# GoatWu/AdaLog

Hardware: AMD Instinct MI355X
Metric: calib_images_per_sec (higher is better)
Workload: dtype bf16

## Files before the change

adalog_amd/csrc/gram.hip:

```cpp
#include "common.h"
#include "fpcs_tail.h"
#include <stdlib.h>
#include <type_traits>
#include <utility>

namespace {

typedef int v4i __attribute__((ext_vector_type(4)));
typedef int v16i __attribute__((ext_vector_type(16)));

template <typename F, int... I> __device__ __forceinline__ void static_for_impl(F&& f, std::integer_sequence<int, I...>) {
    (f(std::integral_constant<int, I>{}), ...);
}
template <int N, typename F> __device__ __forceinline__ void static_for(F&& f) { static_for_impl(f, std::make_integer_sequence<int, N>{}); }

constexpr int RLIMBS = 4;
constexpr int CLIMBS = 8;
constexpr int RFIX_BITS = 29;

__global__ __launch_bounds__(256) void k_gram_pack_xt(const float* __restrict__ x, int T, int K, int64_t ldx, const float* __restrict__ sa,
                                                      const float* __restrict__ za, float qmax, int8_t* __restrict__ xt, int64_t Tp) {
#pragma clang fp contract(off)
    __shared__ uint32_t tile[64][17];
    const int tid = threadIdx.x, tx = tid & 15, ty = tid >> 4;
    const int m0 = blockIdx.x * 64, k0 = blockIdx.y * 64;
    const float s = sa[0], z = rintf(za[0]), inv = 1.0f / s;
#pragma unroll
    for (int i = 0; i < 4; ++i) {
        const int m = m0 + ty + 16 * i, k = k0 + 4 * tx;
        uint32_t pk = 0;
        if (m < T && k < K) {
            const float4 v = *reinterpret_cast<const float4*>(x + (int64_t)m * ldx + k);
            const float e[4] = {v.x, v.y, v.z, v.w};
#pragma unroll
            for (int j = 0; j < 4; ++j) {
                const int q = (int)(uni_bin_fast(e[j], s, inv, z, qmax) - z);
                pk |= ((uint32_t)(q & 0xff)) << (8 * j);
            }
        }
        tile[ty + 16 * i][tx] = pk;
    }
    __syncthreads();
    const int c = tid >> 2, part = tid & 3;
    if (k0 + c < K) {
        uint32_t o[4];
#pragma unroll
        for (int w = 0; w < 4; ++w) {
            uint32_t u = 0;
#pragma unroll
            for (int j = 0; j < 4; ++j) {
                const uint32_t d = tile[part * 16 + w * 4 + j][c >> 2];
                u |= ((d >> (8 * (c & 3))) & 0xffu) << (8 * j);
            }
            o[w] = u;
        }
        *reinterpret_cast<uint4*>(xt + (int64_t)(k0 + c) * Tp + m0 + part * 16) = make_uint4(o[0], o[1], o[2], o[3]);
    }
}

__device__ __forceinline__ double block_sum_d(double v, double* sm) {
#pragma unroll
    for (int o = 32; o > 0; o >>= 1) v += __shfl_xor(v, o);
    const int w = threadIdx.x >> 6;
    __syncthreads();
    if ((threadIdx.x & 63) == 0) sm[w] = v;
    __syncthreads();
    return (sm[0] + sm[1]) + (sm[2] + sm[3]);
}

__global__ __launch_bounds__(256) void k_gram_rmax(const float* __restrict__ ref_t, int T, int chunk, const float* __restrict__ bias,
                                                   unsigned int* __restrict__ amax) {
#pragma clang fp contract(off)
    __shared__ float smf[4];
    const int o = blockIdx.x, tid = threadIdx.x;
    const int m0 = blockIdx.y * chunk, m1 = min(T, m0 + chunk);
    const float* r = ref_t + (int64_t)o * T;
    const float b = bias ? bias[o] : 0.0f;
    float am = 0.0f;
    for (int m = m0 + tid; m < m1; m += 256) am = fmaxf(am, fabsf(r[m] - b));
#pragma unroll
    for (int d = 32; d > 0; d >>= 1) am = fmaxf(am, __shfl_xor(am, d));
    if ((tid & 63) == 0) smf[tid >> 6] = am;
    __syncthreads();
    if (tid == 0) {
        am = fmaxf(fmaxf(smf[0], smf[1]), fmaxf(smf[2], smf[3]));
        if (am == am) atomicMax(amax + o, __float_as_uint(am));
    }
}

__global__ __launch_bounds__(256) void k_gram_rfix(const float* __restrict__ ref_t, int T, int64_t Tp, int O, int chunk, int nchunk,
                                                   const float* __restrict__ bias, const unsigned int* __restrict__ amax,
                                                   int8_t* __restrict__ rl, double* __restrict__ s0p, double* __restrict__ cscl) {
#pragma clang fp contract(off)
    __shared__ double smd[4];
    const int o = blockIdx.x, tid = threadIdx.x;
    const int m0 = blockIdx.y * chunk, m1 = (int)min((int64_t)Tp, (int64_t)m0 + chunk);
    const float* r = ref_t + (int64_t)o * T;
    const float b = bias ? bias[o] : 0.0f;
    const float am = __uint_as_float(amax[o]);
    int e = 0;
    if (am > 0.0f && am < 3.0e38f) e = RFIX_BITS - ilogbf(am);
    const double sc = ldexp(1.0, e);
    double acc = 0.0;
    int8_t* l0 = rl + (int64_t)o * Tp;
    const int64_t plane = (int64_t)O * Tp;
    for (int m = m0 + tid; m < m1; m += 256) {
        int v = 0;
        if (m < T) v = (int)rint((double)(r[m] - b) * sc);
        acc += (double)v * (double)v;
        int rest = v;
#pragma unroll
        for (int l = 0; l < RLIMBS; ++l) {
            const int d = (int)(int8_t)(rest & 0xff);
            l0[l * plane + m] = (int8_t)d;
            rest = (rest - d) >> 8;
        }
    }
    const double tot = block_sum_d(acc, smd);
    if (tid == 0) {
        s0p[(int64_t)o * nchunk + blockIdx.y] = ldexp(tot, -2 * e);
        if (blockIdx.y == 0) cscl[o] = ldexp(1.0, -e);
    }
}

#include "gram_mm.inc"

__global__ __launch_bounds__(256) void k_gram_fin_g(const int* __restrict__ part, int splits, int K, int NL, int8_t* __restrict__ gfrag) {
    const int64_t idx = (int64_t)blockIdx.x * 256 + threadIdx.x;
    if (idx >= (int64_t)K * K) return;
    const int col = (int)(idx % K), slot = (int)(idx / K);
    const int kt = slot >> 5, rp = slot & 31;
    const int row = 32 * kt + 16 * ((rp >> 2) & 1) + 4 * (rp >> 3) + (rp & 3);
    long long g = 0;
    for (int z = 0; z < splits; ++z) g += (long long)part[((int64_t)z * K + row) * K + col];
    const int nj = K >> 5, jt = col >> 5, h = (col >> 4) & 1, e = col & 15;
    long long rest = g;
    for (int l = 0; l < NL; ++l) {
        const int d = (int)(int8_t)(rest & 0xff);
        gfrag[((((int64_t)l * nj + kt) * nj + jt) * 64 + (rp + 32 * h)) * 16 + e] = (int8_t)d;
        rest = (rest - d) >> 8;
    }
}

__global__ __launch_bounds__(256) void k_gram_fin_c(const int* __restrict__ part, int splits, int O, int K, int8_t* __restrict__ clim,
                                                    const double* __restrict__ s0p, int nchunk, double* __restrict__ s0) {
    const int64_t idx = (int64_t)blockIdx.x * 256 + threadIdx.x;
    if (idx < O) {
        double t = 0.0;
        for (int ch = 0; ch < nchunk; ++ch) t += s0p[idx * nchunk + ch];
        s0[idx] = t;
    }
    if (idx >= (int64_t)O * K) return;
    const int o = (int)(idx / K), k = (int)(idx % K);
    long long c = 0;
    for (int z = 0; z < splits; ++z)
#pragma unroll
        for (int l = 0; l < RLIMBS; ++l) c += ((long long)part[((int64_t)z * RLIMBS * O + (int64_t)l * O + o) * K + k]) << (8 * l);
    long long rest = c;
#pragma unroll
    for (int l = 0; l < CLIMBS; ++l) {
        const int d = (int)(int8_t)(rest & 0xff);
        clim[((int64_t)o * CLIMBS + l) * K + k] = (int8_t)d;
        rest = (rest - d) >> 8;
    }
}

template <int OFF> __device__ __forceinline__ v4i gram_rd(uint32_t addr) {
    v4i r;
    asm volatile("ds_read_b128 %0, %1 offset:%2" : "=v"(r) : "v"(addr), "n"(OFF));
    return r;
}
template <int OFF> __device__ __forceinline__ v4i gram_rd_after(uint32_t addr, v16i& tie) {
    v4i r;
    asm volatile("ds_read_b128 %0, %2 offset:%3" : "=v"(r), "+v"(tie) : "v"(addr), "n"(OFF));
    return r;
}
template <int N> __device__ __forceinline__ void gram_wait(v4i& f) {
    if constexpr (N >= 2) asm volatile("s_waitcnt lgkmcnt(2)" : "+v"(f));
    else if constexpr (N == 1) asm volatile("s_waitcnt lgkmcnt(1)" : "+v"(f));
    else asm volatile("s_waitcnt lgkmcnt(0)" : "+v"(f));
}

struct GramScoreArgs {
    const float* W; int64_t ldw; int O, K, P;
    const float* scale; const float* zp;
    const int8_t* gfrag; int NL;
    const int8_t* clim;
    const double* s0; const double* cscl;
    const float* sa;
    double norm;
    float qmax, tie;
    float* scores;
    int nblk;
    long long* timeline;
};

template <int NJ, int NB, bool BIG, bool TIE, int COOP = -1>
__device__ __forceinline__ void gram_pass(const GramScoreArgs& p, uint8_t* lds, int blk0, int w, int lane, float sa, int stamp_slot) {
    constexpr bool CO = COOP >= 0;
    constexpr int QN = CO ? NJ / 4 : NJ;
    constexpr int J0 = CO ? COOP * (NJ / 4) : 0;
    static_assert(!CO || (NJ % 4 == 0 && NB >= 1), "the cooperative pass splits NJ four ways");
    constexpr int NPW = (NJ + 3) / 4;
    constexpr int NRING = 4;
    constexpr int NBA = NB > 0 ? NB : 1;
    const int c = lane & 31, h = lane >> 5;
    const int PB = p.P >> 5;
    const int npanel = NJ * p.NL;
#define GRAM_STAMP(i_) do { if (p.timeline && stamp_slot >= 0 && w == 0 && lane == 0) p.timeline[stamp_slot * 8 + (i_)] = (long long)__builtin_readcyclecounter(); } while (0)
    GRAM_STAMP(0);

    v4i bf[NBA][NJ];
    int orow[NBA];
    float sig[NBA];
    uint8_t* stage = lds + (CO ? 0 : w * (NJ * 1024)) + lane * 16;
    __syncthreads();
    {
#pragma clang fp contract(off)
        static_for<NB>([&](auto bc) {
            constexpr int b = decltype(bc)::value;
            const int blk = blk0 + b;
            const int o = blk / PB, cand = (blk - o * PB) * 32 + c;
            orow[b] = o;
            const int64_t gpi = (int64_t)cand * p.O + o;
            const float gs = p.scale[gpi], gz = rintf(p.zp[gpi]);
            sig[b] = sa * gs;
            const float ginv = __builtin_amdgcn_rcpf(gs);
            const float glo = 128.0f - gz, ghi = 128.0f + (p.qmax - gz);
            const float* __restrict__ wr = p.W + (int64_t)o * p.ldw + 16 * h;
            uint8_t* stb = stage + (CO ? b * (NJ * 1024) : 0);
            float4 nx[4];
#pragma unroll
            for (int j = 0; j < 4; ++j) nx[j] = *reinterpret_cast<const float4*>(wr + 32 * J0 + 4 * j);
#pragma unroll 1
            for (int jt = J0; jt < J0 + QN; ++jt) {
                float xv[16];
#pragma unroll
                for (int j = 0; j < 4; ++j) { xv[4 * j] = nx[j].x; xv[4 * j + 1] = nx[j].y; xv[4 * j + 2] = nx[j].z; xv[4 * j + 3] = nx[j].w; }
                {
                    const int jn = min(jt + 1, NJ - 1);
#pragma unroll
                    for (int j = 0; j < 4; ++j) nx[j] = *reinterpret_cast<const float4*>(wr + 32 * jn + 4 * j);
                }
                float kq[16], dm = 0.0f;
#pragma unroll
                for (int e = 0; e < 16; ++e) {
                    const float t = xv[e] * ginv;
                    kq[e] = rintf(t);
                    dm = fmaxf(dm, fabsf(t - kq[e]));
                }
                if (__builtin_expect(dm > p.tie, 0)) {
#pragma unroll
                    for (int e = 0; e < 16; ++e) kq[e] = rintf(xv[e] / gs);
                }
                v4i pk;
#pragma unroll
                for (int j = 0; j < 4; ++j) {
                    int u = 0;
#pragma unroll
                    for (int e = 0; e < 4; ++e)
                        u = sdwa_rne_byte(u, __builtin_amdgcn_fmed3f(kq[4 * j + e], glo - 128.0f, ghi - 128.0f), 12582912.0f, e);
                    pk[j] = u;
                }
                *reinterpret_cast<v4i*>(stb + jt * 1024) = pk;
            }
            if constexpr (!CO)
                static_for<NJ>([&](auto jtc) { bf[b][decltype(jtc)::value] = *reinterpret_cast<const v4i*>(stb + decltype(jtc)::value * 1024); });
        });
        if constexpr (CO) {
            __syncthreads();
            static_for<NB>([&](auto bc) {
                constexpr int b = decltype(bc)::value;
                static_for<NJ>([&](auto jtc) {
                    bf[b][decltype(jtc)::value] = *reinterpret_cast<const v4i*>(stage + (b * NJ + decltype(jtc)::value) * 1024);
                });
            });
        }
    }
    GRAM_STAMP(1);

    double lin[NBA];
    static_for<NB>([&](auto bc) {
        constexpr int b = decltype(bc)::value;
        v16i acc;
#pragma unroll
        for (int e = 0; e < 16; ++e) acc[e] = 0;
        const int8_t* cr = p.clim + ((int64_t)orow[b] * CLIMBS + (c & 7)) * p.K + 16 * h;
        static_for<QN>([&](auto jtc) {
            constexpr int jt = J0 + decltype(jtc)::value;
            v4i a = *reinterpret_cast<const v4i*>(cr + 32 * jt);
            if (c >= CLIMBS) a = v4i{0, 0, 0, 0};
            acc = __builtin_amdgcn_mfma_i32_32x32x32_i8(a, bf[b][jt], acc, 0, 0, 0);
        });
        double v = 0.0;
#pragma unroll
        for (int j = 0; j < 4; ++j) v += (double)acc[j] * (h ? 4294967296.0 : 1.0) * (double)(1 << (8 * j));
        v += __shfl_xor(v, 32);
        lin[b] = v;
    });
    GRAM_STAMP(2);

    double quad[NBA];
#pragma unroll
    for (int b = 0; b < NBA; ++b) quad[b] = 0.0;
    v4i stg[NPW];
    auto fetch = [&](int pn) {
        const int pc = min(pn, npanel - 1);
        const int8_t* src = p.gfrag + (int64_t)pc * NJ * 1024;
#pragma unroll
        for (int i = 0; i < NPW; ++i) {
            const int piece = min(w + 4 * i, NJ - 1);
            stg[i] = *reinterpret_cast<const v4i*>(src + (int64_t)piece * 1024 + lane * 16);
        }
    };
    auto stash = [&](int pn) {
        uint8_t* dst = lds + (pn % NRING) * (NJ * 1024);
#pragma unroll
        for (int i = 0; i < NPW; ++i) {
            const int piece = min(w + 4 * i, NJ - 1);
            *reinterpret_cast<v4i*>(dst + piece * 1024 + lane * 16) = stg[i];
        }
    };
    __syncthreads();
    fetch(0); stash(0);
    fetch(1); stash(1);
    fetch(2);
    int kt = 0;
    double sh = 1.0;
#pragma unroll 1
    for (int pn = 0; pn < npanel; ++pn) {
        __syncthreads();
        if (pn + 2 < npanel) stash(pn + 2);
        fetch(pn + 3);
        if constexpr (NB > 0) {
            const uint8_t* pan = lds + (pn % NRING) * (NJ * 1024) + lane * 16;
            v16i acc[NB];
#pragma unroll
            for (int b = 0; b < NB; ++b)
#pragma unroll
                for (int e = 0; e < 16; ++e) acc[b][e] = 0;
            constexpr int AD = QN < 3 ? QN : 3;
            v4i af[AD];
            const uint32_t pa = (uint32_t)(uintptr_t)pan;
            static_for<AD>([&](auto ic) { af[decltype(ic)::value] = gram_rd<(J0 + decltype(ic)::value) * 1024>(pa); });
            static_for<QN>([&](auto jtc) {
                constexpr int ji = decltype(jtc)::value, jt = J0 + ji;
                constexpr int left = (QN - 1 - ji) < (AD - 1) ? (QN - 1 - ji) : (AD - 1);
                gram_wait<left>(af[ji % AD]);
                static_for<NB>([&](auto bc) {
                    constexpr int b = decltype(bc)::value;
                    acc[b] = __builtin_amdgcn_mfma_i32_32x32x32_i8(af[ji % AD], bf[b][jt], acc[b], 0, 0, 0);
                });
                if constexpr (ji + AD < QN) {
                    if constexpr (TIE) af[ji % AD] = gram_rd_after<(jt + AD) * 1024>(pa, acc[NB - 1]);
                    else af[ji % AD] = gram_rd<(jt + AD) * 1024>(pa);
                }
            });
            static_for<NB>([&](auto bc) {
                constexpr int b = decltype(bc)::value;
                v4i wv = bf[b][0];
                switch (kt) {
#define GRAM_CASE(i_) case i_: if constexpr ((i_) < NJ) wv = bf[b][(i_) < NJ ? (i_) : 0]; break;
                    GRAM_CASE(1) GRAM_CASE(2) GRAM_CASE(3) GRAM_CASE(4) GRAM_CASE(5) GRAM_CASE(6) GRAM_CASE(7) GRAM_CASE(8)
                    GRAM_CASE(9) GRAM_CASE(10) GRAM_CASE(11) GRAM_CASE(12) GRAM_CASE(13) GRAM_CASE(14) GRAM_CASE(15) GRAM_CASE(16)
                    GRAM_CASE(17) GRAM_CASE(18) GRAM_CASE(19) GRAM_CASE(20) GRAM_CASE(21) GRAM_CASE(22) GRAM_CASE(23)
#undef GRAM_CASE
                    default: break;
                }
                constexpr int GRP = BIG ? 4 : 16;
#pragma unroll
                for (int g0 = 0; g0 < 16; g0 += GRP) {
                    int ts = 0;
#pragma unroll
                    for (int e = g0; e < g0 + GRP; ++e) {
                        const int we = __builtin_amdgcn_sbfe(wv[e >> 2], 8 * (e & 3), 8);
                        ts += __mul24(acc[b][e], we);
                    }
                    quad[b] += (double)ts * sh;
                }
            });
        }
        if (++kt == NJ) { kt = 0; sh *= 256.0; }
    }
    GRAM_STAMP(3);

    if constexpr (CO) {
        double* red = reinterpret_cast<double*>(lds);
        __syncthreads();
        static_for<NB>([&](auto bc) {
            constexpr int b = decltype(bc)::value;
            red[((w * NB + b) * 2 + 0) * 64 + lane] = quad[b];
            red[((w * NB + b) * 2 + 1) * 64 + lane] = lin[b];
        });
        __syncthreads();
        if (w == 0) {
            static_for<NB>([&](auto bc) {
                constexpr int b = decltype(bc)::value;
                double q = 0.0, l = 0.0;
#pragma unroll
                for (int ww = 0; ww < 4; ++ww) { q += red[((ww * NB + b) * 2 + 0) * 64 + lane]; l += red[((ww * NB + b) * 2 + 1) * 64 + lane]; }
                quad[b] = q; lin[b] = l;
            });
        }
    }
    if (!CO || w == 0) {
        static_for<NB>([&](auto bc) {
            constexpr int b = decltype(bc)::value;
            const double q = quad[b] + __shfl_xor(quad[b], 32);
            const int o = orow[b];
            const double s = (double)sig[b];
            const double tot = p.s0[o] - 2.0 * s * (lin[b] * p.cscl[o]) + s * s * q;
            const int blk = blk0 + b;
            const int cand = (blk - o * PB) * 32 + c;
            if (h == 0) p.scores[(int64_t)cand * p.O + o] = (float)(-p.norm * tot);
        });
    }
    GRAM_STAMP(4);
#undef GRAM_STAMP
}

template <int NJ, int CB, bool BIG, int WGS_PER_CU>
__global__ __launch_bounds__(256, WGS_PER_CU) void k_gram_score(GramScoreArgs p) {
#if defined(__HIP_DEVICE_COMPILE__)
    extern __shared__ __attribute__((aligned(16))) uint8_t lds[];
    const int tid = threadIdx.x, lane = tid & 63;
    const int w = __builtin_amdgcn_readfirstlane(tid >> 6);
    const int nwg = gridDim.x;
    const int b_begin = (int)(((int64_t)p.nblk * blockIdx.x) / nwg), b_end = (int)(((int64_t)p.nblk * (blockIdx.x + 1)) / nwg);
    const float sa = p.sa[0];
    int pass_no = 0;
    for (int pass0 = b_begin; pass0 < b_end; pass0 += 4 * CB, ++pass_no) {
        const int n = min(4 * CB, b_end - pass0);
        const int slot = pass_no < 2 ? (int)blockIdx.x * 2 + pass_no : -1;
        if constexpr (NJ % 4 == 0 && NJ >= 8 && NJ != 16) {
            if (n <= CB) {
#define GRAM_COOP(NBV)                                                                                            \
                do {                                                                                              \
                    if (w == 0) gram_pass<NJ, NBV, BIG, WGS_PER_CU == 2, 0>(p, lds, pass0, w, lane, sa, slot);     \
                    else if (w == 1) gram_pass<NJ, NBV, BIG, WGS_PER_CU == 2, 1>(p, lds, pass0, w, lane, sa, slot); \
                    else if (w == 2) gram_pass<NJ, NBV, BIG, WGS_PER_CU == 2, 2>(p, lds, pass0, w, lane, sa, slot); \
                    else gram_pass<NJ, NBV, BIG, WGS_PER_CU == 2, 3>(p, lds, pass0, w, lane, sa, slot);            \
                } while (0)
                if (n == 1) GRAM_COOP(1);
                else if (CB >= 2 && n == 2) GRAM_COOP((CB >= 2 ? 2 : 1));
                else if (CB >= 3 && n == 3) GRAM_COOP((CB >= 3 ? 3 : 1));
                else if (CB >= 4 && n == 4) GRAM_COOP((CB >= 4 ? 4 : 1));
#undef GRAM_COOP
                continue;
            }
        }
        const int nbw = n / 4 + (w < (n & 3) ? 1 : 0);
        const int blk0 = pass0 + w * (n / 4) + min(w, n & 3);
        if (nbw == CB) gram_pass<NJ, CB, BIG, WGS_PER_CU == 2>(p, lds, blk0, w, lane, sa, slot);
        else if (nbw == 0) gram_pass<NJ, 0, BIG, WGS_PER_CU == 2>(p, lds, blk0, w, lane, sa, slot);
        else if (nbw == 1) gram_pass<NJ, 1, BIG, WGS_PER_CU == 2>(p, lds, blk0, w, lane, sa, slot);
        else if (CB > 2 && nbw == 2) gram_pass<NJ, (CB > 2 ? 2 : 1), BIG, WGS_PER_CU == 2>(p, lds, blk0, w, lane, sa, slot);
        else if (CB > 3 && nbw == 3) gram_pass<NJ, (CB > 3 ? 3 : 1), BIG, WGS_PER_CU == 2>(p, lds, blk0, w, lane, sa, slot);
    }
#endif
}

struct GramPlan {
    int T, O, K, NJ, NL;
    int64_t Tp;
    int steps_total, sg_steps, sg_splits, sc_steps, sc_splits, r_chunk, r_nchunk;
    int64_t off_gfrag, off_clim, off_s0, off_cscl, off_xt, off_rl, off_gpart, off_cpart, off_amax, off_s0p, total;
    bool ok;
};

static int g_limbs(int64_t T, int a_bits) {
    const double gmax = (double)T * (double)((1 << a_bits) - 1) * (double)((1 << a_bits) - 1);
    double cover = 127.0;
    for (int L = 1; L <= 7; ++L) {
        if (gmax <= cover) return L;
        cover = cover * 256.0 + 127.0;
    }
    return 8;
}

__global__ __launch_bounds__(256) void k_gram_sum_g(const int* __restrict__ part, int splits, int K, long long* __restrict__ gsum) {
    const int64_t idx = (int64_t)blockIdx.x * 256 + threadIdx.x;
    if (idx >= (int64_t)K * K) return;
    long long g = 0;
    for (int z = 0; z < splits; ++z) g += (long long)part[(int64_t)z * K * K + idx];
    gsum[idx] = g;
}

__global__ __launch_bounds__(256) void k_gram_sum_c(const int* __restrict__ part, int splits, int O, int K, long long* __restrict__ csum,
                                                    const double* __restrict__ s0p, int nchunk, double* __restrict__ s0) {
    const int64_t idx = (int64_t)blockIdx.x * 256 + threadIdx.x;
    if (idx < O) {
        double t = 0.0;
        for (int ch = 0; ch < nchunk; ++ch) t += s0p[idx * nchunk + ch];
        s0[idx] = t;
    }
    if (idx >= (int64_t)O * K) return;
    const int o = (int)(idx / K), k = (int)(idx % K);
    long long c = 0;
    for (int z = 0; z < splits; ++z)
#pragma unroll
        for (int l = 0; l < RLIMBS; ++l) c += ((long long)part[((int64_t)z * RLIMBS * O + (int64_t)l * O + o) * K + k]) << (8 * l);
    csum[idx] = c;
}

__global__ __launch_bounds__(256) void k_gram_limbs_g(const long long* __restrict__ gsum, int K, int NL, int8_t* __restrict__ gfrag) {
    const int64_t idx = (int64_t)blockIdx.x * 256 + threadIdx.x;
    if (idx >= (int64_t)K * K) return;
    const int col = (int)(idx % K), slot = (int)(idx / K);
    const int kt = slot >> 5, rp = slot & 31;
    const int row = 32 * kt + 16 * ((rp >> 2) & 1) + 4 * (rp >> 3) + (rp & 3);
    const int nj = K >> 5, jt = col >> 5, h = (col >> 4) & 1, e = col & 15;
    long long rest = gsum[(int64_t)row * K + col];
    for (int l = 0; l < NL; ++l) {
        const int d = (int)(int8_t)(rest & 0xff);
        gfrag[((((int64_t)l * nj + kt) * nj + jt) * 64 + (rp + 32 * h)) * 16 + e] = (int8_t)d;
        rest = (rest - d) >> 8;
    }
}

__global__ __launch_bounds__(256) void k_gram_limbs_c(const long long* __restrict__ csum, int O, int K, int8_t* __restrict__ clim,
                                                      const double* __restrict__ s0_in, const unsigned int* __restrict__ amax,
                                                      double* __restrict__ s0, double* __restrict__ cscl) {
    const int64_t idx = (int64_t)blockIdx.x * 256 + threadIdx.x;
    if (idx < O) {
        s0[idx] = s0_in[idx];
        const float am = __uint_as_float(amax[idx]);
        int e = 0;
        if (am > 0.0f && am < 3.0e38f) e = RFIX_BITS - ilogbf(am);
        cscl[idx] = ldexp(1.0, -e);
    }
    if (idx >= (int64_t)O * K) return;
    const int o = (int)(idx / K), k = (int)(idx % K);
    long long rest = csum[idx];
#pragma unroll
    for (int l = 0; l < CLIMBS; ++l) {
        const int d = (int)(int8_t)(rest & 0xff);
        clim[((int64_t)o * CLIMBS + l) * K + k] = (int8_t)d;
        rest = (rest - d) >> 8;
    }
}

static int64_t al256(int64_t v) { return (v + 255) / 256 * 256; }

static int pick_steps(int steps_total, int tiles, int target_waves) {
    int splits = (target_waves + tiles - 1) / tiles;
    if (splits < 1) splits = 1;
    int per = (steps_total + splits - 1) / splits;
    if (per < 4) per = 4;
    if (per > 512) per = 512;
    if (per > steps_total) per = steps_total;
    return per;
}

constexpr int MM_BI = 4, MM_BJ = 4;

static GramPlan gram_plan(int T, int O, int K, int a_bits) {
    GramPlan g{};
    g.T = T; g.O = O; g.K = K;
    g.ok = T >= 1 && O >= 1 && K >= 32 && K % 32 == 0 && a_bits >= 2 && a_bits <= 7 && (int64_t)RLIMBS * O < ((int64_t)1 << 30);
    if (!g.ok) return g;
    g.NJ = K / 32;
    g.NL = g_limbs(T, a_bits);
    g.Tp = ((int64_t)T + 127) / 128 * 128;
    g.steps_total = (int)(g.Tp / 128);
    const int tk = (K + 32 * MM_BJ - 1) / (32 * MM_BJ);
    const int tg = ((K + 32 * MM_BI - 1) / (32 * MM_BI)) * tk, tc = ((RLIMBS * O + 32 * MM_BI - 1) / (32 * MM_BI)) * tk;
    g.sg_steps = pick_steps(g.steps_total, tg, 512);
    g.sg_splits = (g.steps_total + g.sg_steps - 1) / g.sg_steps;
    g.sc_steps = pick_steps(g.steps_total, tc, 512);
    g.sc_splits = (g.steps_total + g.sc_steps - 1) / g.sc_steps;
    g.r_chunk = 8192;
    g.r_nchunk = (int)((g.Tp + g.r_chunk - 1) / g.r_chunk);
    int64_t off = 0;
    g.off_gfrag = off; off += al256((int64_t)g.NL * K * K);
    g.off_clim = off; off += al256((int64_t)O * CLIMBS * K);
    g.off_s0 = off; off += al256((int64_t)O * 8);
    g.off_cscl = off; off += al256((int64_t)O * 8);
    g.off_amax = off; off += al256((int64_t)O * 4);
    g.off_s0p = off; off += al256((int64_t)O * g.r_nchunk * 8);
    g.off_xt = off; off += al256((int64_t)K * g.Tp);
    g.off_rl = off; off += al256((int64_t)RLIMBS * O * g.Tp);
    g.off_gpart = off; off += al256((int64_t)g.sg_splits * K * K * 4);
    g.off_cpart = off; off += al256((int64_t)g.sc_splits * RLIMBS * O * K * 4);
    g.total = off;
    return g;
}

static bool nj_supported(int nj) { return nj == 1 || nj == 2 || nj == 3 || nj == 4 || nj == 6 || nj == 8 || nj == 12 || nj == 16 || nj == 24; }

}

extern "C" int adalog_gram_supported(int T, int O, int K, int a_bits, int w_bits, int P) {
    const GramPlan g = gram_plan(T, O, K, a_bits);
    if (!g.ok || !nj_supported(g.NJ) || w_bits < 2 || w_bits > 7 || P < 32 || P % 32 != 0) return 0;
    const int64_t wq = (1 << w_bits) - 1;
    if ((int64_t)128 * wq * K >= (1 << 23)) return 0;
    if ((w_bits > 4 ? 4 : 16) * 128 * wq * wq * K >= ((int64_t)1 << 31)) return 0;
    if ((int64_t)O * P / 32 >= ((int64_t)1 << 30)) return 0;
    return 1;
}

extern "C" int adalog_gram_ok(int T, int O, int K, int a_bits, int w_bits, int P) {
    if (!adalog_gram_supported(T, O, K, a_bits, w_bits, P)) return 0;
    return (int64_t)g_limbs(T, a_bits) * K * 2 <= T ? 1 : 0;
}

extern "C" int adalog_gram_limbs(int T, int a_bits) { return (T >= 1 && a_bits >= 2 && a_bits <= 7) ? g_limbs(T, a_bits) : -1; }

extern "C" int64_t adalog_gram_workspace_bytes(int T, int O, int K, int a_bits) {
    const GramPlan g = gram_plan(T, O, K, a_bits);
    return g.ok ? g.total : -1;
}

extern "C" int adalog_gram_build(const float* x, int T, int K, int64_t ldx, const float* sa, const float* za, int a_bits,
                                 const float* ref_t, int O, const float* bias, void* ws, int64_t ws_bytes, void* stream) {
    ADALOG_ARG_CHECK(x && sa && za && ref_t && ws, "gram_build: null pointer");
    const GramPlan g = gram_plan(T, O, K, a_bits);
    ADALOG_ARG_CHECK(g.ok && nj_supported(g.NJ), "gram_build: shape not supported (adalog_gram_supported)");
    ADALOG_ARG_CHECK(ws_bytes >= g.total, "gram_build: workspace too small");
    ADALOG_ARG_CHECK(ldx >= K && ldx % 4 == 0 && ((uintptr_t)x & 15) == 0 && ((uintptr_t)ws & 255) == 0, "gram_build: x rows / workspace must be aligned");
    hipStream_t st = (hipStream_t)stream;
    uint8_t* base = (uint8_t*)ws;
    int8_t* xt = (int8_t*)(base + g.off_xt);
    int8_t* rl = (int8_t*)(base + g.off_rl);
    int* gpart = (int*)(base + g.off_gpart);
    int* cpart = (int*)(base + g.off_cpart);
    unsigned int* amax = (unsigned int*)(base + g.off_amax);
    double* s0p = (double*)(base + g.off_s0p);
    {
        const hipError_t me = hipMemsetAsync(amax, 0, (size_t)O * 4, st);
        if (me != hipSuccess) { adalog_set_error("adalog_gram_build (clear)", me); return (int)me; }
    }
    hipLaunchKernelGGL(k_gram_pack_xt, dim3((unsigned)(g.Tp / 64), (unsigned)((K + 63) / 64)), dim3(256), 0, st, x, T, K, ldx, sa, za,
                       (float)((1 << a_bits) - 1), xt, g.Tp);
    hipLaunchKernelGGL(k_gram_rmax, dim3((unsigned)O, (unsigned)g.r_nchunk), dim3(256), 0, st, ref_t, T, g.r_chunk, bias, amax);
    hipLaunchKernelGGL(k_gram_rfix, dim3((unsigned)O, (unsigned)g.r_nchunk), dim3(256), 0, st, ref_t, T, g.Tp, O, g.r_chunk, g.r_nchunk, bias,
                       amax, rl, s0p, (double*)(base + g.off_cscl));
    const unsigned tk = (unsigned)((K + 32 * MM_BJ - 1) / (32 * MM_BJ));
    hipLaunchKernelGGL(k_i8mm, dim3((unsigned)((K + 32 * MM_BI - 1) / (32 * MM_BI)), tk, (unsigned)g.sg_splits), dim3(256), 0, st,
                       xt, xt, K, K, g.Tp, g.sg_steps, g.steps_total, gpart);
    hipLaunchKernelGGL(k_i8mm, dim3((unsigned)((RLIMBS * O + 32 * MM_BI - 1) / (32 * MM_BI)), tk, (unsigned)g.sc_splits), dim3(256), 0,
                       st, rl, xt, RLIMBS * O, K, g.Tp, g.sc_steps, g.steps_total, cpart);
    hipLaunchKernelGGL(k_gram_fin_g, dim3((unsigned)(((int64_t)K * K + 255) / 256)), dim3(256), 0, st, gpart, g.sg_splits, K, g.NL,
                       (int8_t*)(base + g.off_gfrag));
    hipLaunchKernelGGL(k_gram_fin_c, dim3((unsigned)(((int64_t)O * K + 255) / 256)), dim3(256), 0, st, cpart, g.sc_splits, O, K,
                       (int8_t*)(base + g.off_clim), s0p, g.r_nchunk, (double*)(base + g.off_s0));
    ADALOG_LAUNCH_CHECK("adalog_gram_build");
    return 0;
}

extern "C" int adalog_gram_amax(const float* ref_t, int T, int O, const float* bias, unsigned int* amax, void* stream) {
    ADALOG_ARG_CHECK(ref_t && amax && T >= 1 && O >= 1, "gram_amax: bad arguments");
    hipStream_t st = (hipStream_t)stream;
    const hipError_t me = hipMemsetAsync(amax, 0, (size_t)O * 4, st);
    if (me != hipSuccess) { adalog_set_error("adalog_gram_amax (clear)", me); return (int)me; }
    const int chunk = 8192, nchunk = (T + chunk - 1) / chunk;
    hipLaunchKernelGGL(k_gram_rmax, dim3((unsigned)O, (unsigned)nchunk), dim3(256), 0, st, ref_t, T, chunk, bias, amax);
    ADALOG_LAUNCH_CHECK("adalog_gram_amax");
    return 0;
}

extern "C" int adalog_gram_build_sums(const float* x, int T, int K, int64_t ldx, const float* sa, const float* za, int a_bits,
                                      const float* ref_t, int O, const float* bias, const unsigned int* amax, long long* gsum,
                                      long long* csum, double* s0, void* ws, int64_t ws_bytes, void* stream) {
    ADALOG_ARG_CHECK(x && sa && za && ref_t && amax && gsum && csum && s0 && ws, "gram_build_sums: null pointer");
    const GramPlan g = gram_plan(T, O, K, a_bits);
    ADALOG_ARG_CHECK(g.ok, "gram_build_sums: shape not supported");
    ADALOG_ARG_CHECK(ws_bytes >= g.total, "gram_build_sums: workspace too small (adalog_gram_workspace_bytes of the LOCAL shape)");
    ADALOG_ARG_CHECK(ldx >= K && ldx % 4 == 0 && ((uintptr_t)x & 15) == 0 && ((uintptr_t)ws & 255) == 0, "gram_build_sums: x rows / workspace must be aligned");
    hipStream_t st = (hipStream_t)stream;
    uint8_t* base = (uint8_t*)ws;
    int8_t* xt = (int8_t*)(base + g.off_xt);
    int8_t* rl = (int8_t*)(base + g.off_rl);
    int* gpart = (int*)(base + g.off_gpart);
    int* cpart = (int*)(base + g.off_cpart);
    double* s0p = (double*)(base + g.off_s0p);
    hipLaunchKernelGGL(k_gram_pack_xt, dim3((unsigned)(g.Tp / 64), (unsigned)((K + 63) / 64)), dim3(256), 0, st, x, T, K, ldx, sa, za,
                       (float)((1 << a_bits) - 1), xt, g.Tp);
    hipLaunchKernelGGL(k_gram_rfix, dim3((unsigned)O, (unsigned)g.r_nchunk), dim3(256), 0, st, ref_t, T, g.Tp, O, g.r_chunk, g.r_nchunk, bias,
                       amax, rl, s0p, (double*)(base + g.off_cscl));
    const unsigned tk = (unsigned)((K + 32 * MM_BJ - 1) / (32 * MM_BJ));
    hipLaunchKernelGGL(k_i8mm, dim3((unsigned)((K + 32 * MM_BI - 1) / (32 * MM_BI)), tk, (unsigned)g.sg_splits), dim3(256), 0, st,
                       xt, xt, K, K, g.Tp, g.sg_steps, g.steps_total, gpart);
    hipLaunchKernelGGL(k_i8mm, dim3((unsigned)((RLIMBS * O + 32 * MM_BI - 1) / (32 * MM_BI)), tk, (unsigned)g.sc_splits), dim3(256), 0,
                       st, rl, xt, RLIMBS * O, K, g.Tp, g.sc_steps, g.steps_total, cpart);
    hipLaunchKernelGGL(k_gram_sum_g, dim3((unsigned)(((int64_t)K * K + 255) / 256)), dim3(256), 0, st, gpart, g.sg_splits, K, gsum);
    hipLaunchKernelGGL(k_gram_sum_c, dim3((unsigned)(((int64_t)O * K + 255) / 256)), dim3(256), 0, st, cpart, g.sc_splits, O, K, csum,
                       s0p, g.r_nchunk, s0);
    ADALOG_LAUNCH_CHECK("adalog_gram_build_sums");
    return 0;
}

extern "C" int adalog_gram_build_from_sums(const long long* gsum, const long long* csum, const double* s0, const unsigned int* amax,
                                           int T_total, int O, int K, int a_bits, void* ws, int64_t ws_bytes, void* stream) {
    ADALOG_ARG_CHECK(gsum && csum && s0 && amax && ws, "gram_build_from_sums: null pointer");
    const GramPlan g = gram_plan(T_total, O, K, a_bits);
    ADALOG_ARG_CHECK(g.ok && nj_supported(g.NJ), "gram_build_from_sums: shape not supported (adalog_gram_supported)");
    ADALOG_ARG_CHECK(ws_bytes >= g.total && ((uintptr_t)ws & 255) == 0, "gram_build_from_sums: workspace too small / misaligned");
    hipStream_t st = (hipStream_t)stream;
    uint8_t* base = (uint8_t*)ws;
    hipLaunchKernelGGL(k_gram_limbs_g, dim3((unsigned)(((int64_t)K * K + 255) / 256)), dim3(256), 0, st, gsum, K, g.NL,
                       (int8_t*)(base + g.off_gfrag));
    hipLaunchKernelGGL(k_gram_limbs_c, dim3((unsigned)(((int64_t)O * K + 255) / 256)), dim3(256), 0, st, csum, O, K,
                       (int8_t*)(base + g.off_clim), s0, amax, (double*)(base + g.off_s0), (double*)(base + g.off_cscl));
    ADALOG_LAUNCH_CHECK("adalog_gram_build_from_sums");
    return 0;
}

static long long* g_gram_timeline = nullptr;
extern "C" void adalog_gram_set_timeline(long long* buf) { g_gram_timeline = buf; }

static int device_cus_gram() { return adalog_device_cus(); }

extern "C" int adalog_gram_score_w(const float* W, int O, int K, int64_t ldw, const float* scale, const float* zp, int P, int w_bits,
                                   const void* ws, int T, int a_bits, const float* sa, double norm, float* scores, void* stream) {
    ADALOG_ARG_CHECK(W && scale && zp && ws && sa && scores, "gram_score_w: null pointer");
    ADALOG_ARG_CHECK(adalog_gram_supported(T, O, K, a_bits, w_bits, P), "gram_score_w: shape not supported (adalog_gram_supported)");
    ADALOG_ARG_CHECK(ldw >= K && ldw % 4 == 0 && ((uintptr_t)W & 15) == 0, "gram_score_w: weight rows must be 16-byte aligned");
    const GramPlan g = gram_plan(T, O, K, a_bits);
    ADALOG_ARG_CHECK(g.ok && nj_supported(g.NJ) && P % 32 == 0, "gram_score_w: shape not supported");
    const uint8_t* base = (const uint8_t*)ws;
    GramScoreArgs a{};
    a.W = W; a.ldw = ldw; a.O = O; a.K = K; a.P = P; a.scale = scale; a.zp = zp;
    a.gfrag = (const int8_t*)(base + g.off_gfrag); a.NL = g.NL; a.clim = (const int8_t*)(base + g.off_clim);
    a.s0 = (const double*)(base + g.off_s0); a.cscl = (const double*)(base + g.off_cscl);
    a.sa = sa; a.norm = norm; a.scores = scores;
    a.qmax = (float)((1 << w_bits) - 1);
    const float zone = 6e-7f * (float)(1 << w_bits);
    a.tie = 0.5f - (zone > 1e-5f ? zone : 1e-5f);
    a.nblk = (int)((int64_t)O * P / 32);
    a.timeline = g_gram_timeline;
    const bool big = w_bits > 4;
    hipStream_t st = (hipStream_t)stream;
    const int ncu = device_cus_gram();
    const int rc = adalog_dispatch<1, 2, 3, 4, 6, 8, 12, 16, 24>(g.NJ, [&](auto nj) {
        return adalog_dispatch<true, false>(big, [&](auto bg) {
            constexpr int NJ = decltype(nj)::value, CB = NJ >= 8 ? 2 : 4, WPC = NJ == 24 ? 1 : 2;
            const int wgs = a.nblk < WPC * ncu ? a.nblk : WPC * ncu;
            return adalog_launch<k_gram_score<NJ, CB, decltype(bg)::value, WPC>>("k_gram_score<i8>", 160 * 1024, (unsigned)wgs, 256,
                                                                                 (size_t)4 * NJ * 1024, st, a);
        });
    });
    if (rc) return rc;
    ADALOG_LAUNCH_CHECK("adalog_gram_score_w");
    return 0;
}

extern "C" int adalog_gram_score_w_tail(const float* W, int O, int K, int64_t ldw, const float* scale, const float* zp, int P, int w_bits,
                                        const void* ws, int T, int a_bits, const float* sa, double norm, float* scores,
                                        const adalog_fpcs_tail* tail, void* stream) {
    const char* why = fpcs::tail_problem(tail, P);
    ADALOG_ARG_CHECK(why == nullptr, why);
    const int rc = adalog_gram_score_w(W, O, K, ldw, scale, zp, P, w_bits, ws, T, a_bits, sa, norm, scores, stream);
    if (rc || !tail) return rc;
    return adalog_topk_next_tail(scores, P, O, tail, nullptr, stream);
}
```

Measured before the change: 38.11.

## Stream Gram panels via buffer-to-LDS DMA in grouped double buffers

Result: slower. 37.69 (-1.1%).

```diff
diff --git a/adalog_amd/csrc/gram.hip b/adalog_amd/csrc/gram.hip
--- a/adalog_amd/csrc/gram.hip
+++ b/adalog_amd/csrc/gram.hip
@@ -8,6 +8,7 @@
 
 typedef int v4i __attribute__((ext_vector_type(4)));
 typedef int v16i __attribute__((ext_vector_type(16)));
+typedef void __attribute__((address_space(3)))* las_ptr;
 
 template <typename F, int... I> __device__ __forceinline__ void static_for_impl(F&& f, std::integer_sequence<int, I...>) {
     (f(std::integral_constant<int, I>{}), ...);
@@ -195,7 +196,7 @@
     long long* timeline;
 };
 
-template <int NJ, int NB, bool BIG, bool TIE, int COOP = -1>
+template <int NJ, int NB, bool BIG, bool TIE, int G, int COOP = -1>
 __device__ __forceinline__ void gram_pass(const GramScoreArgs& p, uint8_t* lds, int blk0, int w, int lane, float sa, int stamp_slot) {
     constexpr bool CO = COOP >= 0;
     constexpr int QN = CO ? NJ / 4 : NJ;
@@ -303,84 +304,185 @@
     double quad[NBA];
 #pragma unroll
     for (int b = 0; b < NBA; ++b) quad[b] = 0.0;
-    v4i stg[NPW];
-    auto fetch = [&](int pn) {
-        const int pc = min(pn, npanel - 1);
-        const int8_t* src = p.gfrag + (int64_t)pc * NJ * 1024;
-#pragma unroll
-        for (int i = 0; i < NPW; ++i) {
-            const int piece = min(w + 4 * i, NJ - 1);
-            stg[i] = *reinterpret_cast<const v4i*>(src + (int64_t)piece * 1024 + lane * 16);
-        }
-    };
-    auto stash = [&](int pn) {
-        uint8_t* dst = lds + (pn % NRING) * (NJ * 1024);
-#pragma unroll
-        for (int i = 0; i < NPW; ++i) {
-            const int piece = min(w + 4 * i, NJ - 1);
-            *reinterpret_cast<v4i*>(dst + piece * 1024 + lane * 16) = stg[i];
-        }
-    };
-    __syncthreads();
-    fetch(0); stash(0);
-    fetch(1); stash(1);
-    fetch(2);
-    int kt = 0;
-    double sh = 1.0;
+    if constexpr (G == 0) {
+        v4i stg[NPW];
+        auto fetch = [&](int pn) {
+            const int pc = min(pn, npanel - 1);
+            const int8_t* src = p.gfrag + (int64_t)pc * NJ * 1024;
+#pragma unroll
+            for (int i = 0; i < NPW; ++i) {
+                const int piece = min(w + 4 * i, NJ - 1);
+                stg[i] = *reinterpret_cast<const v4i*>(src + (int64_t)piece * 1024 + lane * 16);
+            }
+        };
+        auto stash = [&](int pn) {
+            uint8_t* dst = lds + (pn % NRING) * (NJ * 1024);
+#pragma unroll
+            for (int i = 0; i < NPW; ++i) {
+                const int piece = min(w + 4 * i, NJ - 1);
+                *reinterpret_cast<v4i*>(dst + piece * 1024 + lane * 16) = stg[i];
+            }
+        };
+        __syncthreads();
+        fetch(0); stash(0);
+        fetch(1); stash(1);
+        fetch(2);
+        int kt = 0;
+        double sh = 1.0;
 #pragma unroll 1
-    for (int pn = 0; pn < npanel; ++pn) {
-        __syncthreads();
-        if (pn + 2 < npanel) stash(pn + 2);
-        fetch(pn + 3);
-        if constexpr (NB > 0) {
-            const uint8_t* pan = lds + (pn % NRING) * (NJ * 1024) + lane * 16;
-            v16i acc[NB];
-#pragma unroll
-            for (int b = 0; b < NB; ++b)
-#pragma unroll
-                for (int e = 0; e < 16; ++e) acc[b][e] = 0;
-            constexpr int AD = QN < 3 ? QN : 3;
-            v4i af[AD];
-            const uint32_t pa = (uint32_t)(uintptr_t)pan;
-            static_for<AD>([&](auto ic) { af[decltype(ic)::value] = gram_rd<(J0 + decltype(ic)::value) * 1024>(pa); });
-            static_for<QN>([&](auto jtc) {
-                constexpr int ji = decltype(jtc)::value, jt = J0 + ji;
-                constexpr int left = (QN - 1 - ji) < (AD - 1) ? (QN - 1 - ji) : (AD - 1);
-                gram_wait<left>(af[ji % AD]);
+        for (int pn = 0; pn < npanel; ++pn) {
+#if !defined(GRAM_LAB_NOBAR)
+            __syncthreads();
+#endif
+#if !defined(GRAM_LAB_NOLOAD)
+            if (pn + 2 < npanel) stash(pn + 2);
+            fetch(pn + 3);
+#endif
+            if constexpr (NB > 0) {
+                const uint8_t* pan = lds + (pn % NRING) * (NJ * 1024) + lane * 16;
+                v16i acc[NB];
+#pragma unroll
+                for (int b = 0; b < NB; ++b)
+#pragma unroll
+                    for (int e = 0; e < 16; ++e) acc[b][e] = 0;
+                constexpr int AD = QN < 3 ? QN : 3;
+                v4i af[AD];
+                const uint32_t pa = (uint32_t)(uintptr_t)pan;
+                static_for<AD>([&](auto ic) { af[decltype(ic)::value] = gram_rd<(J0 + decltype(ic)::value) * 1024>(pa); });
+                static_for<QN>([&](auto jtc) {
+                    constexpr int ji = decltype(jtc)::value, jt = J0 + ji;
+                    constexpr int left = (QN - 1 - ji) < (AD - 1) ? (QN - 1 - ji) : (AD - 1);
+                    gram_wait<left>(af[ji % AD]);
+                    static_for<NB>([&](auto bc) {
+                        constexpr int b = decltype(bc)::value;
+                        acc[b] = __builtin_amdgcn_mfma_i32_32x32x32_i8(af[ji % AD], bf[b][jt], acc[b], 0, 0, 0);
+                    });
+                    if constexpr (ji + AD < QN) {
+                        if constexpr (TIE) af[ji % AD] = gram_rd_after<(jt + AD) * 1024>(pa, acc[NB - 1]);
+                        else af[ji % AD] = gram_rd<(jt + AD) * 1024>(pa);
+                    }
+                });
                 static_for<NB>([&](auto bc) {
                     constexpr int b = decltype(bc)::value;
-                    acc[b] = __builtin_amdgcn_mfma_i32_32x32x32_i8(af[ji % AD], bf[b][jt], acc[b], 0, 0, 0);
+#if defined(GRAM_LAB_NODOT)
+                    quad[b] += (double)acc[b][0] * sh;
+                    return;
+#endif
+                    v4i wv = bf[b][0];
+                    switch (kt) {
+#define GRAM_CASE(i_) case i_: if constexpr ((i_) < NJ) wv = bf[b][(i_) < NJ ? (i_) : 0]; break;
+                        GRAM_CASE(1) GRAM_CASE(2) GRAM_CASE(3) GRAM_CASE(4) GRAM_CASE(5) GRAM_CASE(6) GRAM_CASE(7) GRAM_CASE(8)
+                        GRAM_CASE(9) GRAM_CASE(10) GRAM_CASE(11) GRAM_CASE(12) GRAM_CASE(13) GRAM_CASE(14) GRAM_CASE(15) GRAM_CASE(16)
+                        GRAM_CASE(17) GRAM_CASE(18) GRAM_CASE(19) GRAM_CASE(20) GRAM_CASE(21) GRAM_CASE(22) GRAM_CASE(23)
+#undef GRAM_CASE
+                        default: break;
+                    }
+                    constexpr int GRP = BIG ? 4 : 16;
+#pragma unroll
+                    for (int g0 = 0; g0 < 16; g0 += GRP) {
+                        int ts = 0;
+#pragma unroll
+                        for (int e = g0; e < g0 + GRP; ++e) {
+                            const int we = __builtin_amdgcn_sbfe(wv[e >> 2], 8 * (e & 3), 8);
+                            ts += __mul24(acc[b][e], we);
+                        }
+                        quad[b] += (double)ts * sh;
+                    }
                 });
-                if constexpr (ji + AD < QN) {
-                    if constexpr (TIE) af[ji % AD] = gram_rd_after<(jt + AD) * 1024>(pa, acc[NB - 1]);
-                    else af[ji % AD] = gram_rd<(jt + AD) * 1024>(pa);
-                }
+            }
+            if (++kt == NJ) { kt = 0; sh *= 256.0; }
+        }
+    } else {
+        int kt = 0;
+        double sh = 1.0;
+        auto panel = [&](const uint8_t* pan, auto&& between) {
+            if constexpr (NB > 0) {
+                v16i acc[NB];
+#pragma unroll
+                for (int b = 0; b < NB; ++b)
+#pragma unroll
+                    for (int e = 0; e < 16; ++e) acc[b][e] = 0;
+                constexpr int AD = QN < 3 ? QN : 3;
+                v4i af[AD];
+                const uint32_t pa = (uint32_t)(uintptr_t)pan;
+                static_for<AD>([&](auto ic) { af[decltype(ic)::value] = gram_rd<(J0 + decltype(ic)::value) * 1024>(pa); });
+                static_for<QN>([&](auto jtc) {
+                    constexpr int ji = decltype(jtc)::value, jt = J0 + ji;
+                    constexpr int left = (QN - 1 - ji) < (AD - 1) ? (QN - 1 - ji) : (AD - 1);
+                    gram_wait<left>(af[ji % AD]);
+                    static_for<NB>([&](auto bc) {
+                        constexpr int b = decltype(bc)::value;
+                        acc[b] = __builtin_amdgcn_mfma_i32_32x32x32_i8(af[ji % AD], bf[b][jt], acc[b], 0, 0, 0);
+                    });
+                    if constexpr (ji + AD < QN) {
+                        if constexpr (TIE) af[ji % AD] = gram_rd_after<(jt + AD) * 1024>(pa, acc[NB - 1]);
+                        else af[ji % AD] = gram_rd<(jt + AD) * 1024>(pa);
+                    }
+                    between(jtc);
+                });
+                static_for<NB>([&](auto bc) {
+                    constexpr int b = decltype(bc)::value;
+                    v4i wv = bf[b][0];
+                    switch (kt) {
+#define GRAM_CASE(i_) case i_: if constexpr ((i_) < NJ) wv = bf[b][(i_) < NJ ? (i_) : 0]; break;
+                        GRAM_CASE(1) GRAM_CASE(2) GRAM_CASE(3) GRAM_CASE(4) GRAM_CASE(5) GRAM_CASE(6) GRAM_CASE(7) GRAM_CASE(8)
+                        GRAM_CASE(9) GRAM_CASE(10) GRAM_CASE(11) GRAM_CASE(12) GRAM_CASE(13) GRAM_CASE(14) GRAM_CASE(15) GRAM_CASE(16)
+                        GRAM_CASE(17) GRAM_CASE(18) GRAM_CASE(19) GRAM_CASE(20) GRAM_CASE(21) GRAM_CASE(22) GRAM_CASE(23)
+#undef GRAM_CASE
+                        default: break;
+                    }
+                    constexpr int GRP = BIG ? 4 : 16;
+#pragma unroll
+                    for (int g0 = 0; g0 < 16; g0 += GRP) {
+                        int ts = 0;
+#pragma unroll
+                        for (int e = g0; e < g0 + GRP; ++e) {
+                            const int we = __builtin_amdgcn_sbfe(wv[e >> 2], 8 * (e & 3), 8);
+                            ts += __mul24(acc[b][e], we);
+                        }
+                        quad[b] += (double)ts * sh;
+                    }
+                });
+            }
+        };
+        static_assert(NJ % G == 0, "a group of panels stays within one limb");
+        constexpr int GPIECES = G * NJ, GBYTES = GPIECES * 1024;
+        constexpr int NPG = (GPIECES + 3) / 4;
+        const int ngroup = npanel / G;
+        const auto rg = __builtin_amdgcn_make_buffer_rsrc((void*)p.gfrag, 0, npanel * NJ * 1024, 0x00020000);
+        auto dma = [&](int g, int i) {
+            const int piece = w + 4 * i;
+            if (GPIECES % 4 == 0 || piece < GPIECES)
+                __builtin_amdgcn_raw_ptr_buffer_load_lds(rg, (las_ptr)(lds + (g & 1) * GBYTES + piece * 1024), 16, lane * 16,
+                                                         g * GBYTES + piece * 1024, 0, 0);
+        };
+        __syncthreads();
+#pragma unroll
+        for (int i = 0; i < NPG; ++i) dma(0, i);
+#pragma unroll 1
+        for (int g = 0; g < ngroup; ++g) {
+            asm volatile("s_waitcnt vmcnt(0)" ::: "memory");
+            __syncthreads();
+            const bool more = g + 1 < ngroup;
+            if constexpr (NB == 0) {
+                if (more)
+#pragma unroll
+                    for (int i = 0; i < NPG; ++i) dma(g + 1, i);
+            }
+            static_for<G>([&](auto sc) {
+                constexpr int s = decltype(sc)::value;
+                panel(lds + (g & 1) * GBYTES + s * (NJ * 1024) + lane * 16, [&](auto jtc) {
+                    constexpr int i = s * QN + decltype(jtc)::value;
+                    if constexpr (i < NPG) { if (more) dma(g + 1, i); }
+                });
+                if (++kt == NJ) { kt = 0; sh *= 256.0; }
             });
-            static_for<NB>([&](auto bc) {
-                constexpr int b = decltype(bc)::value;
-                v4i wv = bf[b][0];
-                switch (kt) {
-#define GRAM_CASE(i_) case i_: if constexpr ((i_) < NJ) wv = bf[b][(i_) < NJ ? (i_) : 0]; break;
-                    GRAM_CASE(1) GRAM_CASE(2) GRAM_CASE(3) GRAM_CASE(4) GRAM_CASE(5) GRAM_CASE(6) GRAM_CASE(7) GRAM_CASE(8)
-                    GRAM_CASE(9) GRAM_CASE(10) GRAM_CASE(11) GRAM_CASE(12) GRAM_CASE(13) GRAM_CASE(14) GRAM_CASE(15) GRAM_CASE(16)
-                    GRAM_CASE(17) GRAM_CASE(18) GRAM_CASE(19) GRAM_CASE(20) GRAM_CASE(21) GRAM_CASE(22) GRAM_CASE(23)
-#undef GRAM_CASE
-                    default: break;
-                }
-                constexpr int GRP = BIG ? 4 : 16;
-#pragma unroll
-                for (int g0 = 0; g0 < 16; g0 += GRP) {
-                    int ts = 0;
-#pragma unroll
-                    for (int e = g0; e < g0 + GRP; ++e) {
-                        const int we = __builtin_amdgcn_sbfe(wv[e >> 2], 8 * (e & 3), 8);
-                        ts += __mul24(acc[b][e], we);
-                    }
-                    quad[b] += (double)ts * sh;
-                }
-            });
+            if constexpr (NB > 0 && NPG > G * QN) {
+                if (more)
+#pragma unroll
+                    for (int i = G * QN; i < NPG; ++i) dma(g + 1, i);
+            }
         }
-        if (++kt == NJ) { kt = 0; sh *= 256.0; }
     }
     GRAM_STAMP(3);
 
@@ -419,7 +521,7 @@
 #undef GRAM_STAMP
 }
 
-template <int NJ, int CB, bool BIG, int WGS_PER_CU>
+template <int NJ, int CB, bool BIG, int WGS_PER_CU, int G>
 __global__ __launch_bounds__(256, WGS_PER_CU) void k_gram_score(GramScoreArgs p) {
 #if defined(__HIP_DEVICE_COMPILE__)
     extern __shared__ __attribute__((aligned(16))) uint8_t lds[];
@@ -436,10 +538,10 @@
             if (n <= CB) {
 #define GRAM_COOP(NBV)                                                                                            \
                 do {                                                                                              \
-                    if (w == 0) gram_pass<NJ, NBV, BIG, WGS_PER_CU == 2, 0>(p, lds, pass0, w, lane, sa, slot);     \
-                    else if (w == 1) gram_pass<NJ, NBV, BIG, WGS_PER_CU == 2, 1>(p, lds, pass0, w, lane, sa, slot); \
-                    else if (w == 2) gram_pass<NJ, NBV, BIG, WGS_PER_CU == 2, 2>(p, lds, pass0, w, lane, sa, slot); \
-                    else gram_pass<NJ, NBV, BIG, WGS_PER_CU == 2, 3>(p, lds, pass0, w, lane, sa, slot);            \
+                    if (w == 0) gram_pass<NJ, NBV, BIG, WGS_PER_CU == 2, G, 0>(p, lds, pass0, w, lane, sa, slot);     \
+                    else if (w == 1) gram_pass<NJ, NBV, BIG, WGS_PER_CU == 2, G, 1>(p, lds, pass0, w, lane, sa, slot); \
+                    else if (w == 2) gram_pass<NJ, NBV, BIG, WGS_PER_CU == 2, G, 2>(p, lds, pass0, w, lane, sa, slot); \
+                    else gram_pass<NJ, NBV, BIG, WGS_PER_CU == 2, G, 3>(p, lds, pass0, w, lane, sa, slot);            \
                 } while (0)
                 if (n == 1) GRAM_COOP(1);
                 else if (CB >= 2 && n == 2) GRAM_COOP((CB >= 2 ? 2 : 1));
@@ -451,11 +553,11 @@
         }
         const int nbw = n / 4 + (w < (n & 3) ? 1 : 0);
         const int blk0 = pass0 + w * (n / 4) + min(w, n & 3);
-        if (nbw == CB) gram_pass<NJ, CB, BIG, WGS_PER_CU == 2>(p, lds, blk0, w, lane, sa, slot);
-        else if (nbw == 0) gram_pass<NJ, 0, BIG, WGS_PER_CU == 2>(p, lds, blk0, w, lane, sa, slot);
-        else if (nbw == 1) gram_pass<NJ, 1, BIG, WGS_PER_CU == 2>(p, lds, blk0, w, lane, sa, slot);
-        else if (CB > 2 && nbw == 2) gram_pass<NJ, (CB > 2 ? 2 : 1), BIG, WGS_PER_CU == 2>(p, lds, blk0, w, lane, sa, slot);
-        else if (CB > 3 && nbw == 3) gram_pass<NJ, (CB > 3 ? 3 : 1), BIG, WGS_PER_CU == 2>(p, lds, blk0, w, lane, sa, slot);
+        if (nbw == CB) gram_pass<NJ, CB, BIG, WGS_PER_CU == 2, G>(p, lds, blk0, w, lane, sa, slot);
+        else if (nbw == 0) gram_pass<NJ, 0, BIG, WGS_PER_CU == 2, G>(p, lds, blk0, w, lane, sa, slot);
+        else if (nbw == 1) gram_pass<NJ, 1, BIG, WGS_PER_CU == 2, G>(p, lds, blk0, w, lane, sa, slot);
+        else if (CB > 2 && nbw == 2) gram_pass<NJ, (CB > 2 ? 2 : 1), BIG, WGS_PER_CU == 2, G>(p, lds, blk0, w, lane, sa, slot);
+        else if (CB > 3 && nbw == 3) gram_pass<NJ, (CB > 3 ? 3 : 1), BIG, WGS_PER_CU == 2, G>(p, lds, blk0, w, lane, sa, slot);
     }
 #endif
 }
@@ -586,6 +688,13 @@
     return g;
 }
 
+#if defined(GRAM_LAB_GROUP)
+constexpr int gram_group(int nj) { return (nj % GRAM_LAB_GROUP == 0 && 2 * GRAM_LAB_GROUP * nj <= (nj == 24 ? 160 : 80)) ? GRAM_LAB_GROUP : 0; }
+#else
+constexpr int gram_group(int nj) { return nj == 12 ? 3 : 0; }
+#endif
+constexpr size_t gram_lds_bytes(int nj, int g) { return (size_t)(g > 2 ? 2 * g : 4) * nj * 1024; }
+
 static bool nj_supported(int nj) { return nj == 1 || nj == 2 || nj == 3 || nj == 4 || nj == 6 || nj == 8 || nj == 12 || nj == 16 || nj == 24; }
 
 }
@@ -733,12 +842,21 @@
     const bool big = w_bits > 4;
     hipStream_t st = (hipStream_t)stream;
     const int ncu = device_cus_gram();
+    const char* sched_env = getenv("ADALOG_GRAM_SCORE_SCHED");
+    const bool grouped = !(sched_env && sched_env[0] == '0');
     const int rc = adalog_dispatch<1, 2, 3, 4, 6, 8, 12, 16, 24>(g.NJ, [&](auto nj) {
         return adalog_dispatch<true, false>(big, [&](auto bg) {
             constexpr int NJ = decltype(nj)::value, CB = NJ >= 8 ? 2 : 4, WPC = NJ == 24 ? 1 : 2;
             const int wgs = a.nblk < WPC * ncu ? a.nblk : WPC * ncu;
-            return adalog_launch<k_gram_score<NJ, CB, decltype(bg)::value, WPC>>("k_gram_score<i8>", 160 * 1024, (unsigned)wgs, 256,
-                                                                                 (size_t)4 * NJ * 1024, st, a);
+            auto launch = [&](auto gc) {
+                constexpr int G = decltype(gc)::value;
+                return adalog_launch<k_gram_score<NJ, CB, decltype(bg)::value, WPC, G>>("k_gram_score<i8>", 160 * 1024, (unsigned)wgs, 256,
+                                                                                        gram_lds_bytes(NJ, G), st, a);
+            };
+            if constexpr (gram_group(NJ) > 0) {
+                if (grouped) return launch(std::integral_constant<int, gram_group(NJ)>{});
+            }
+            return launch(std::integral_constant<int, 0>{});
         });
     });
     if (rc) return rc;
```
